# jianing-sun/Mask-YOLO

Measured on AMD Instinct MI355X. Metric: images/sec fwd+bwd, 224x224 Shapes batch 32, at 1 MI355X, higher is better.
Workload: dtype f32

## Files before the change

mask-yolo_amd/csrc/mem_kernels.hip:

```cpp
#include "myolo_common.h"
#include <type_traits>
#include <stdlib.h>
#include <stdarg.h>
#include <string.h>

static thread_local char g_err[512] = "";
extern "C" void myolo_set_error(const char* fmt, ...)
{
    va_list ap;
    va_start(ap, fmt);
    vsnprintf(g_err, sizeof(g_err), fmt, ap);
    va_end(ap);
}
extern "C" const char* myolo_last_error_string(void) { return g_err; }
extern "C" int myolo_version(void) { return 213; }

static MyoloOptions default_options() { MyoloOptions o = {}; o.bn_fused_tf_variance = 1; o.tn_wgs = 224; return o; }
MyoloOptions g_myolo_opt = default_options();
static int* option_slot(const char* name)
{
    static const struct { const char* n; int MyoloOptions::*m; } tab[] = {
        {"gemm_generic", &MyoloOptions::gemm_generic}, {"no_splitk", &MyoloOptions::no_splitk}, {"bf16_no256", &MyoloOptions::bf16_no256},
        {"bf16_force256", &MyoloOptions::bf16_force256}, {"bf16_no_c3", &MyoloOptions::bf16_no_c3}, {"bf16_no_loopn", &MyoloOptions::bf16_no_loopn},
        {"bf16_mask_valu", &MyoloOptions::bf16_mask_valu}, {"bf16_mask_nofin", &MyoloOptions::bf16_mask_nofin},
        {"deconv_mask_legacy", &MyoloOptions::deconv_mask_legacy}, {"crop_bf16_legacy", &MyoloOptions::crop_bf16_legacy},
        {"tune0", &MyoloOptions::tune0}, {"wino_x6", &MyoloOptions::wino_x6}, {"wino_no_bt", &MyoloOptions::wino_no_bt},
        {"wino_no_mixed", &MyoloOptions::wino_no_mixed}, {"x6_no_half_tiles", &MyoloOptions::x6_no_half_tiles},
        {"w63_legacy", &MyoloOptions::w63_legacy}, {"pw_x6_min_rows", &MyoloOptions::pw_x6_min_rows}, {"deconv_no_x6", &MyoloOptions::deconv_no_x6},
        {"pw_no_smallm", &MyoloOptions::pw_no_smallm}, {"pw_no_x6", &MyoloOptions::pw_no_x6}, {"tn_no_x6", &MyoloOptions::tn_no_x6},
        {"tn_wgs", &MyoloOptions::tn_wgs}, {"tn_x6_legacy", &MyoloOptions::tn_x6_legacy}, {"no_trunk_fusion", &MyoloOptions::no_trunk_fusion},
        {"bn_fused_tf_variance", &MyoloOptions::bn_fused_tf_variance},
    };
    if (!name) return nullptr;
    for (const auto& e : tab)
        if (strcmp(e.n, name) == 0) return &(g_myolo_opt.*(e.m));
    return nullptr;
}
extern "C" int myolo_set_option(const char* name, int value)
{
    int* s = option_slot(name);
    MYOLO_REQUIRE(s, "set_option: unknown option '%s'", name ? name : "(null)");
    *s = value;
    return MYOLO_OK;
}
extern "C" int myolo_get_option(const char* name, int* value)
{
    int* s = option_slot(name);
    MYOLO_REQUIRE(s && value, "get_option: unknown option '%s'", name ? name : "(null)");
    *value = *s;
    return MYOLO_OK;
}

#include <vector>
struct WPrepEntry {
    const void* w; int kind; long long d0, d1, d2;
    size_t off, bytes;
    unsigned long long gen;
    unsigned long long last_use;
    std::function<void(void*, hipStream_t)> run;
};
struct WPrep {
    char* arena; size_t cap, used;
    unsigned long long gen;
// ... 3439 lines not shown
```

mask-yolo_amd/csrc/myolo_common.h:

```cpp
#pragma once
#include <hip/hip_runtime.h>
#include <stdint.h>
#include <stdio.h>
#include "../../include/myolo_hip_internal.h"

extern "C" void myolo_set_error(const char* fmt, ...);

struct MyoloOptions {
    int gemm_generic;
    int no_splitk;
    int bf16_no256;
    int bf16_no_loopn;
    int bf16_mask_valu;
    int bf16_mask_nofin;
    int deconv_mask_legacy;
    int bf16_no_c3;
    int bf16_force256;
    int crop_bf16_legacy;
    int tune0;
    int wino_x6;
    int wino_no_bt;
    int wino_no_mixed;
    int x6_no_half_tiles;
    int w63_legacy;
    int pw_x6_min_rows;
    int deconv_no_x6;
    int pw_no_smallm;
    int pw_no_x6;
    int tn_no_x6;
    int tn_wgs;
    int tn_x6_legacy;
    int no_trunk_fusion;
    int bn_fused_tf_variance;
};
extern MyoloOptions g_myolo_opt;

#define MYOLO_REQUIRE(cond, ...)                                   \
    do {                                                           \
        if (!(cond)) {                                             \
            myolo_set_error(__VA_ARGS__);                          \
            return MYOLO_EINVAL;                                   \
        }                                                          \
    } while (0)

#define MYOLO_NEED_WS(bytes)                                                         \
    do {                                                                             \
        if ((size_t)(bytes) > ws_bytes || (ws == nullptr && (bytes) > 0)) {          \
            myolo_set_error("%s: workspace too small (%zu needed, %zu given)",       \
                            __func__, (size_t)(bytes), ws_bytes);                    \
            return MYOLO_EWORKSPACE;                                                 \
        }                                                                            \
    } while (0)

#define MYOLO_CHECK_LAUNCH()                                                         \
    do {                                                                             \
        hipError_t e__ = hipGetLastError();                                          \
        if (e__ != hipSuccess) {                                                     \
            myolo_set_error("%s: launch failed: %s", __func__, hipGetErrorString(e__)); \
            return MYOLO_ELAUNCH;                                                    \
        }                                                                            \
    } while (0)

#include <functional>
enum { WP_TRANSPOSE = 1, WP_X6_SPLIT = 2, WP_WINO63_U = 3, WP_WINO43_U = 4 };
// ... 47 lines not shown
```

mask-yolo_amd/csrc/wino_mm.hip:

```cpp
#include "myolo_common.h"

typedef float f32x16 __attribute__((ext_vector_type(16)));
typedef unsigned int u32x4 __attribute__((ext_vector_type(4)));

#define MM_BM 128
#define MM_BN 256
#define MM_BK 16
#define MM_LD 20
#define MM_OOB 0x7fffff00u

struct MMRun {
    long long rows;
    long long a_off;
    long long b_off;
    long long c_off;
    long long tile0;
    int mtiles;
    int nq;
};
struct MMArgs {
    const float* A;
    const float* Bt;
    float* C;
    int K, N;
// ... 347 lines not shown
            const long long row = m0 + wm * 64 + t * 32 + (r & 3) + 8 * (r >> 2) + 4 * half;
            if (row >= M) continue;
            float* dst = Cp + row * p.N + n0 + wn * 128 + l31;
#pragma unroll
            for (int u = 0; u < 4; ++u) dst[32 * u] = acc[t][u][r];
        }
}

typedef __bf16 bf16x8 __attribute__((ext_vector_type(8)));
#define X6_REC 112

__device__ __forceinline__ unsigned x6_top(float lo, float hi) { return __builtin_amdgcn_perm(__float_as_uint(hi), __float_as_uint(lo), 0x07060302u); }
__device__ __forceinline__ float x6_rest(float x) { return x - __uint_as_float(__float_as_uint(x) & 0xffff0000u); }
__device__ __forceinline__ bf16x8 x6_ldb(__amdgpu_buffer_rsrc_t r, unsigned voff, unsigned soff)
{
    u32x4 v = __builtin_amdgcn_raw_buffer_load_b128(r, (int)voff, (int)soff, 0);
    return __builtin_bit_cast(bf16x8, v);
}

template <int V> struct IntK { static constexpr int value = V; };
template <bool SWAP> __device__ __forceinline__ f32x16 x6_mfma(bf16x8 a, bf16x8 b, f32x16 c)
{
    if constexpr (SWAP) return __builtin_amdgcn_mfma_f32_32x32x16_bf16(b, a, c, 0, 0, 0);
    else return __builtin_amdgcn_mfma_f32_32x32x16_bf16(a, b, c, 0, 0, 0);
}

__device__ __forceinline__ float mm_act(float v, int act)
{
    if (act == MYOLO_ACT_RELU) return fmaxf(v, 0.f);
    if (act == MYOLO_ACT_RELU6) return fminf(fmaxf(v, 0.f), 6.f);
    return v;
}

template <int EPI, bool PW = false, int AG = MM_A_PLAIN, int NU = 4>
__global__ __launch_bounds__(256, 2) void wino_mm_x6_kernel(MMArgs p)
{
    static_assert(NU == 4 || (NU == 2 && EPI == MM_EP_PLAIN && AG == MM_A_PLAIN), "the 128-column tile exists for the plain product only");
    constexpr int BN = 64 * NU;
    __shared__ __attribute__((aligned(16))) unsigned char As[2][MM_BM * X6_REC];
    __shared__ __attribute__((aligned(16))) unsigned char etab[EPI == MM_EP_DECONV_MASK_T ? 5120 + 4096 : 16];

    const int tid = threadIdx.x, lane = tid & 63, wave = tid >> 6;
    const int wm = wave >> 1, wn = wave & 1, half = lane >> 5, l31 = lane & 31;
    const int ntn = p.N / BN;
    long long bid;
    {
        const long long nwg = gridDim.x, orig = blockIdx.x;
        const long long q = nwg >> 3, r = nwg & 7, xcd = orig & 7;
        bid = (xcd < r ? xcd * (q + 1) : r * (q + 1) + (xcd - r) * q) + (orig >> 3);
    }
    int ri = 0;
#pragma unroll
    for (int k = 1; k < 4; ++k)
        if (k < p.nruns && bid >= p.run[k].tile0) ri = k;
    const MMRun& R = p.run[ri];
    const long long local = bid - R.tile0;
    const long long per_plane = (long long)R.mtiles * ntn;
    const int z = (int)(local / per_plane);
    const long long rem = local - z * per_plane;
    const int n0 = (int)(rem % ntn) * BN;
    const long long m0 = (rem / ntn) * MM_BM;
    const long long M = R.rows;
    const int nk = p.K / MM_BK;
    const float* Ap = p.A + R.a_off + (long long)z * M * p.K;
    const unsigned char* Bp = reinterpret_cast<const unsigned char*>(p.Bt) + (R.b_off + (long long)z * p.K * p.N) * 6;
    float* Cp = p.C + R.c_off + (long long)z * M * p.N;
    const long long mend = (m0 + MM_BM < M) ? m0 + MM_BM : M;
    const int arow = tid >> 1, ah = tid & 1;
    __amdgpu_buffer_rsrc_t ra;
    unsigned aoffg;
    unsigned ag_base = 0;
// ... 3 lines not shown
        ra = mm_rsrc(Ap + base_px * p.Co, (end_px - base_px) * p.Co * 4);
        const long long mm = m0 + arow;
        if (mm < M) {
            const long long hw = (long long)p.H * p.W;
            const int rem = (int)(mm - (mm / hw) * hw);
            const int x = rem - (rem / p.W) * p.W;
            ag_base = (unsigned)((4 * mm - 2 * x - base_px) * p.Co + ah * 8) * 4u;
        } else ag_base = MM_OOB;
        aoffg = ag_base;
    } else {
        ra = mm_rsrc(Ap + m0 * p.K, (mend - m0) * p.K * 4);
        aoffg = ((unsigned)arow * (unsigned)p.K + (unsigned)ah * 8u) * 4u;
    }
    const __amdgpu_buffer_rsrc_t rb = mm_rsrc(reinterpret_cast<const float*>(Bp), (long long)p.K * p.N * 6);
    int ag_k = 0;
    const int asto = arow * X6_REC + ah * 16;
    float4 sa[2];
    float4 psc[2], psh[2];
    int kch = ah * 8;
    auto gload = [&]() {
        if constexpr (AG == MM_A_DECONV) {
            const int tap = ag_k / p.Co, c0 = ag_k - tap * p.Co;
            const unsigned sh = (unsigned)(((tap >> 1) * 2 * p.W + (tap & 1)) * p.Co + c0) * 4u;
            aoffg = ag_base == MM_OOB ? MM_OOB : ag_base + sh;
            ag_k += MM_BK;
        }
        sa[0] = mm_bufld4(ra, aoffg);
        sa[1] = mm_bufld4(ra, aoffg == MM_OOB ? MM_OOB : aoffg + 16u);
#ifdef MM_X6_TUNE
        if constexpr (AG == MM_A_PLAIN) { if (!(p.tune & 16)) aoffg += MM_BK * 4u; }
#else
        if constexpr (AG == MM_A_PLAIN) aoffg += MM_BK * 4u;
#endif
        if (PW && p.a_scale) {
            psc[0] = *reinterpret_cast<const float4*>(p.a_scale + kch); psc[1] = *reinterpret_cast<const float4*>(p.a_scale + kch + 4);
            psh[0] = *reinterpret_cast<const float4*>(p.a_shift + kch); psh[1] = *reinterpret_cast<const float4*>(p.a_shift + kch + 4);
            kch += MM_BK;
        }
    };
    auto affine = [&]() {
        if (PW && p.a_scale) {
            sa[0].x = mm_act(fmaf(sa[0].x, psc[0].x, psh[0].x), p.a_act); sa[0].y = mm_act(fmaf(sa[0].y, psc[0].y, psh[0].y), p.a_act);
            sa[0].z = mm_act(fmaf(sa[0].z, psc[0].z, psh[0].z), p.a_act); sa[0].w = mm_act(fmaf(sa[0].w, psc[0].w, psh[0].w), p.a_act);
            sa[1].x = mm_act(fmaf(sa[1].x, psc[1].x, psh[1].x), p.a_act); sa[1].y = mm_act(fmaf(sa[1].y, psc[1].y, psh[1].y), p.a_act);
            sa[1].z = mm_act(fmaf(sa[1].z, psc[1].z, psh[1].z), p.a_act); sa[1].w = mm_act(fmaf(sa[1].w, psc[1].w, psh[1].w), p.a_act);
        }
    };
    auto sstore = [&](int buf) {
        affine();
        const float x[8] = {sa[0].x, sa[0].y, sa[0].z, sa[0].w, sa[1].x, sa[1].y, sa[1].z, sa[1].w};
        float r1[8], r2[8];
#pragma unroll
        for (int e = 0; e < 8; ++e) { r1[e] = x6_rest(x[e]); r2[e] = x6_rest(r1[e]); }
        u32x4 p1, p2, p3;
#pragma unroll
        for (int e = 0; e < 4; ++e) {
            p1[e] = x6_top(x[2 * e], x[2 * e + 1]);
            p2[e] = x6_top(r1[2 * e], r1[2 * e + 1]);
            p3[e] = x6_top(r2[2 * e], r2[2 * e + 1]);
        }
        *reinterpret_cast<u32x4*>(As[buf] + asto) = p1;
        *reinterpret_cast<u32x4*>(As[buf] + asto + 32) = p2;
        *reinterpret_cast<u32x4*>(As[buf] + asto + 64) = p3;
    };
    const int afr = (wm * 64 + l31) * X6_REC + half * 16;
    const unsigned bvo = (unsigned)(((n0 + wn * 32 * NU) >> 5) * 6 + half) * 512u + (unsigned)l31 * 16u;
    const unsigned bchunk = (unsigned)(p.N >> 5) * 3072u;
    unsigned bso = 0;
    bf16x8 bq[NU][3];

    f32x16 acc[2][NU];
#pragma unroll
    for (int t = 0; t < 2; ++t)
#pragma unroll
        for (int u = 0; u < NU; ++u)
#pragma unroll
            for (int r = 0; r < 16; ++r) acc[t][u][r] = 0.f;

    gload();
#pragma unroll
    for (int u = 0; u < NU; ++u)
#pragma unroll
        for (int pc = 0; pc < 3; ++pc) bq[u][pc] = x6_ldb(rb, bvo + u * 3072u + pc * 1024u, bso);
    sstore(0);
    if (nk > 1) gload();
    if constexpr (EPI == MM_EP_DECONV_MASK_T) mm_deconv_mask_table(p, etab, n0, tid);
    __syncthreads();
    bf16x8 fa[2][3];
#pragma unroll
    for (int pc = 0; pc < 3; ++pc) fa[0][pc] = *reinterpret_cast<const bf16x8*>(As[0] + afr + pc * 32);

    if constexpr (NU == 2 && AG == MM_A_PLAIN && EPI == MM_EP_PLAIN) {
        float4 qa[3][2], qsc[3][2], qsh[3][2];
        bf16x8 qb[2][NU][3];
        const float* csc = (PW && p.a_scale) ? p.a_scale : p.A;
        const float* csh = (PW && p.a_scale) ? p.a_shift : p.A;
        const bool has_aff = PW && p.a_scale;
        auto gstage = [&](auto st, bool valid) {
            constexpr int S = decltype(st)::value;
#ifdef MM_X6_TUNE
            if (!(p.tune & 2048)) {
#endif
            qa[S][0] = mm_bufld4(ra, valid ? aoffg : MM_OOB);
            qa[S][1] = mm_bufld4(ra, valid ? aoffg + 16u : MM_OOB);
#ifdef MM_X6_TUNE
            }
#endif
            aoffg += MM_BK * 4u;
#ifdef MM_X6_TUNE
            if (p.tune & 8192) return;
#endif
            if constexpr (PW) {
                const int kc = (valid && has_aff) ? kch : ah * 8;
                qsc[S][0] = *reinterpret_cast<const float4*>(csc + kc); qsc[S][1] = *reinterpret_cast<const float4*>(csc + kc + 4);
                qsh[S][0] = *reinterpret_cast<const float4*>(csh + kc); qsh[S][1] = *reinterpret_cast<const float4*>(csh + kc + 4);
                kch += MM_BK;
            }
        };
        qa[1][0] = sa[0]; qa[1][1] = sa[1];
        if constexpr (PW) { qsc[1][0] = psc[0]; qsc[1][1] = psc[1]; qsh[1][0] = psh[0]; qsh[1][1] = psh[1]; }
#pragma unroll
        for (int u = 0; u < NU; ++u)
#pragma unroll
            for (int pc = 0; pc < 3; ++pc) {
                qb[0][u][pc] = bq[u][pc];
                qb[1][u][pc] = x6_ldb(rb, bvo + u * 3072u + pc * 1024u, nk > 1 ? bchunk : 0u);
            }
        gstage(IntK<2>{}, nk > 2);
        gstage(IntK<0>{}, nk > 3);
        auto step = [&](auto ic, int c) {
            constexpr int I = decltype(ic)::value;
            constexpr int cur = I & 1, SA = (I + 1) % 3, SB = I & 1;
            const bool more = c + 1 < nk;
#ifdef MM_X6_TUNE
            if (!(p.tune & 16384))
#endif
#pragma unroll
            for (int pc = 0; pc < 3; ++pc) fa[1][pc] = *reinterpret_cast<const bf16x8*>(As[cur] + afr + 32 * X6_REC + pc * 32);
            float x[8] = {qa[SA][0].x, qa[SA][0].y, qa[SA][0].z, qa[SA][0].w, qa[SA][1].x, qa[SA][1].y, qa[SA][1].z, qa[SA][1].w};
            if constexpr (PW) {
                if (has_aff) {
                    const float sc8[8] = {qsc[SA][0].x, qsc[SA][0].y, qsc[SA][0].z, qsc[SA][0].w, qsc[SA][1].x, qsc[SA][1].y, qsc[SA][1].z, qsc[SA][1].w};
                    const float sh8[8] = {qsh[SA][0].x, qsh[SA][0].y, qsh[SA][0].z, qsh[SA][0].w, qsh[SA][1].x, qsh[SA][1].y, qsh[SA][1].z, qsh[SA][1].w};
#pragma unroll
                    for (int e = 0; e < 8; ++e) x[e] = mm_act(fmaf(x[e], sc8[e], sh8[e]), p.a_act);
                }
            }
            gstage(IntK<SA>{}, c + 4 < nk);
            const unsigned b2 = c + 2 < nk ? bso + 2u * bchunk : bso;
            u32x4 p1, p2, p3;
            bf16x8 fn0, fn1, fn2;
#pragma unroll
            for (int u = 0; u < NU; ++u) {
#ifdef MM_X6_TUNE
#define X6_GO (!(p.tune & 512))
#else
#define X6_GO true
#endif
#define X6_TILE(t)  if (X6_GO) {                                                                                         \
                acc[t][u] = __builtin_amdgcn_mfma_f32_32x32x16_bf16(fa[t][0], qb[SB][u][2], acc[t][u], 0, 0, 0);       \
                acc[t][u] = __builtin_amdgcn_mfma_f32_32x32x16_bf16(fa[t][2], qb[SB][u][0], acc[t][u], 0, 0, 0);       \
                acc[t][u] = __builtin_amdgcn_mfma_f32_32x32x16_bf16(fa[t][1], qb[SB][u][1], acc[t][u], 0, 0, 0);       \
                acc[t][u] = __builtin_amdgcn_mfma_f32_32x32x16_bf16(fa[t][0], qb[SB][u][1], acc[t][u], 0, 0, 0);       \
                acc[t][u] = __builtin_amdgcn_mfma_f32_32x32x16_bf16(fa[t][1], qb[SB][u][0], acc[t][u], 0, 0, 0);       \
                acc[t][u] = __builtin_amdgcn_mfma_f32_32x32x16_bf16(fa[t][0], qb[SB][u][0], acc[t][u], 0, 0, 0); }
                X6_TILE(0)
                X6_TILE(1)
#undef X6_TILE
#undef X6_GO
#ifdef MM_X6_TUNE
                if (!(p.tune & 1024))
#endif
#pragma unroll
// ... 25 lines not shown
                    if (more && !(p.tune & 16384)) {
#else
                    if (more) {
#endif
                        fn0 = *reinterpret_cast<const bf16x8*>(As[cur ^ 1] + afr);
                        fn1 = *reinterpret_cast<const bf16x8*>(As[cur ^ 1] + afr + 32);
                        fn2 = *reinterpret_cast<const bf16x8*>(As[cur ^ 1] + afr + 64);
                    }
                }
                __builtin_amdgcn_sched_barrier(0);
            }
            if (more) { fa[0][0] = fn0; fa[0][1] = fn1; fa[0][2] = fn2; }
            bso = more ? bso + bchunk : bso;
        };
        int c0 = 0;
        for (; c0 + 6 <= nk; c0 += 6) {
            step(IntK<0>{}, c0); step(IntK<1>{}, c0 + 1); step(IntK<2>{}, c0 + 2);
            step(IntK<3>{}, c0 + 3); step(IntK<4>{}, c0 + 4); step(IntK<5>{}, c0 + 5);
        }
        if (c0 < nk) step(IntK<0>{}, c0);
        if (c0 + 1 < nk) step(IntK<1>{}, c0 + 1);
        if (c0 + 2 < nk) step(IntK<2>{}, c0 + 2);
        if (c0 + 3 < nk) step(IntK<3>{}, c0 + 3);
        if (c0 + 4 < nk) step(IntK<4>{}, c0 + 4);
    } else
    for (int c = 0; c < nk; ++c) {
        const int cur = c & 1;
        const bool more = c + 1 < nk;
#ifdef MM_X6_TUNE
        if (!(p.tune & 64))
#endif
#pragma unroll
        for (int pc = 0; pc < 3; ++pc) fa[1][pc] = *reinterpret_cast<const bf16x8*>(As[cur] + afr + 32 * X6_REC + pc * 32);
        affine();
        const float x[8] = {sa[0].x, sa[0].y, sa[0].z, sa[0].w, sa[1].x, sa[1].y, sa[1].z, sa[1].w};
        u32x4 p1, p2, p3;
#ifdef MM_X6_TUNE
        if (c + 2 < nk && !(p.tune & 128)) gload();
#else
        if (c + 2 < nk) gload();
#endif
#ifdef MM_X6_TUNE
        const unsigned bnext = (p.tune & 1) ? 0u : (more ? bso + bchunk : bso);
#else
        const unsigned bnext = more ? bso + bchunk : bso;
#endif
        bf16x8 fn0, fn1, fn2;
#pragma unroll
        for (int u = 0; u < NU; ++u) {
#define X6_TILE(t)                                                                                                 \
            if (X6_ALL) {                                                                                          \
            acc[t][u] = x6_mfma<EPI == MM_EP_DECONV_MASK_T>(fa[t][0], bq[u][2], acc[t][u]);           \
            acc[t][u] = x6_mfma<EPI == MM_EP_DECONV_MASK_T>(fa[t][2], bq[u][0], acc[t][u]);           \
            acc[t][u] = x6_mfma<EPI == MM_EP_DECONV_MASK_T>(fa[t][1], bq[u][1], acc[t][u]); }         \
            acc[t][u] = x6_mfma<EPI == MM_EP_DECONV_MASK_T>(fa[t][0], bq[u][1], acc[t][u]);           \
            acc[t][u] = x6_mfma<EPI == MM_EP_DECONV_MASK_T>(fa[t][1], bq[u][0], acc[t][u]);           \
            acc[t][u] = x6_mfma<EPI == MM_EP_DECONV_MASK_T>(fa[t][0], bq[u][0], acc[t][u]);
#ifdef MM_X6_TUNE
#define X6_ALL (!(p.tune & 256))
#else
#define X6_ALL true
#endif
            X6_TILE(0)
            X6_TILE(1)
#undef X6_TILE
#undef X6_ALL
#ifdef MM_X6_TUNE
// ... 315 lines not shown
    }
    MYOLO_CHECK_LAUNCH();
    return MYOLO_OK;
}

#define TN_T 256
struct TNRun {
    long long rows;
    long long a_off, b_off;
    long long rows_per_split;
    long long unit0;
    int plane0;
    int nq;
    int splits;
};
struct TNArgs {
    const float* a_scale;
    const float* a_shift;
    int a_act;
    int gH, gW, gCo;
    const float* A;
    const float* B;
    float* part;
    float* C;
    int Ka, N;
    int nruns;
    int tiles_k, tiles_n;
    long long nunits;
    long long unit_base;
    int tune;
    TNRun run[4];
};

template <bool AG = false, bool UNI = true>
__global__ __launch_bounds__(512, 1) void wino_tn_x6_kernel(TNArgs p)
{
    __shared__ __attribute__((aligned(16))) unsigned char Ls[2][2][TN_T * X6_REC];

    const int tid = threadIdx.x, lane = tid & 63, wave = tid >> 6;
    const int wm = wave >> 2, wn = wave & 3, half = lane >> 5, l31 = lane & 31;
    const int ntile = p.tiles_k * p.tiles_n;
  const long long bid = p.unit_base + blockIdx.x;
  {
    const long long pair = bid / ntile;
    const int tile = (int)(bid - pair * ntile);
    const int kat = tile / p.tiles_n, nt = tile - kat * p.tiles_n;
    int ri = 0;
#pragma unroll
    for (int k = 1; k < 4; ++k)
        if (k < p.nruns && pair >= p.run[k].unit0) ri = k;
    const TNRun& R = p.run[ri];
    const long long local = pair - R.unit0;
    const int z = (int)(local / R.splits), sp = (int)(local - (long long)z * R.splits);
    const long long r0 = (long long)sp * R.rows_per_split;
    long long r1 = r0 + R.rows_per_split;
    if (r1 > R.rows) r1 = R.rows;
    const long long nrows = r1 > r0 ? r1 - r0 : 0;
    const int nk = (int)((nrows + MM_BK - 1) / MM_BK);

    const int op = UNI ? __builtin_amdgcn_readfirstlane(tid >> 8) : tid >> 8, col = tid & 255;
    const int ld = op ? p.N : p.Ka;
    const float* base = op ? p.B + R.b_off + ((long long)z * R.rows + r0) * p.N + nt * TN_T
                           : p.A + R.a_off + ((long long)z * R.rows + r0) * p.Ka + kat * TN_T;
    __amdgpu_buffer_rsrc_t rs = mm_rsrc(base, (nrows * ld - (op ? nt : kat) * TN_T) * 4);
    unsigned voff = (unsigned)col * 4u;
    const unsigned rowb = (unsigned)ld * 4u;
    unsigned soff = 0;
    long long g_m = r0, g_base_px = 0;
    int g_x = 0;
// ... 9 lines not shown
    }
    float st[16];
    auto gload = [&]() {
        if (AG && op == 0) {
            int xk = g_x;
#pragma unroll
            for (int k = 0; k < 16; ++k) {
                const long long m = g_m + k;
                const unsigned so = m < r1 ? (unsigned)((4 * m - 2 * xk - g_base_px) * p.gCo) * 4u : MM_OOB;
                st[k] = __uint_as_float(__builtin_amdgcn_raw_buffer_load_b32(rs, (int)(so == MM_OOB ? MM_OOB : voff + so), 0, 0));
                if (++xk == p.gW) xk = 0;
            }
            g_m += 16;
            g_x = xk;
            return;
        }
#ifdef MM_X6_TUNE
        if (p.tune & 1) {
#pragma unroll
            for (int k = 0; k < 16; ++k) st[k] = __uint_as_float(__builtin_amdgcn_raw_buffer_load_b32(rs, (int)MM_OOB, 0, 0));
            return;
        }
        if (p.tune & 16) {
#pragma unroll
            for (int k = 0; k < 16; ++k) st[k] = __uint_as_float(__builtin_amdgcn_raw_buffer_load_b32(rs, (int)voff, (int)((unsigned)k * rowb), 0));
            return;
        }
#endif
#pragma unroll
        for (int k = 0; k < 16; ++k) st[k] = __uint_as_float(__builtin_amdgcn_raw_buffer_load_b32(rs, (int)voff, (int)(soff + (unsigned)k * rowb), 0));
        soff += 16u * rowb;
    };
    unsigned char* const wbase = &Ls[0][op][col * X6_REC];
    const bool pro = p.a_scale != nullptr && op == 0;
    const float csc = pro ? p.a_scale[kat * TN_T + col] : 1.f, csh = pro ? p.a_shift[kat * TN_T + col] : 0.f;
    long long rows_staged = 0;
    auto split_store = [&](int buf, int h) {
        u32x4 p1, p2, p3;
        if (pro) {
#pragma unroll
            for (int j = 0; j < 8; ++j)
                if (rows_staged + 8 * h + j < nrows) st[8 * h + j] = mm_act(fmaf(st[8 * h + j], csc, csh), p.a_act);
        }
#pragma unroll
        for (int e = 0; e < 4; ++e) {
            const float a0 = st[8 * h + 2 * e], a1 = st[8 * h + 2 * e + 1];
#ifdef MM_X6_TUNE
            if (p.tune & 2) { p1[e] = x6_top(a0, a1); p2[e] = p1[e]; p3[e] = p1[e]; continue; }
#endif
            const float b0 = x6_rest(a0), b1 = x6_rest(a1);
            p1[e] = x6_top(a0, a1);
            p2[e] = x6_top(b0, b1);
            p3[e] = x6_top(x6_rest(b0), x6_rest(b1));
        }
#ifdef MM_X6_TUNE
        if (p.tune & 8) return;
#endif
        unsigned char* w = wbase + buf * (2 * TN_T * X6_REC) + h * 16;
        *reinterpret_cast<u32x4*>(w) = p1;
        *reinterpret_cast<u32x4*>(w + 32) = p2;
        *reinterpret_cast<u32x4*>(w + 64) = p3;
    };
    const int afr = (wm * 128 + l31) * X6_REC + half * 16;
    const int bfr = (wn * 64 + l31) * X6_REC + half * 16;

    f32x16 acc[4][2];
#pragma unroll
    for (int t = 0; t < 4; ++t)
#pragma unroll
        for (int u = 0; u < 2; ++u)
#pragma unroll
            for (int r = 0; r < 16; ++r) acc[t][u][r] = 0.f;

    if (nk > 0) {
        gload();
        split_store(0, 0);
        split_store(0, 1);
        if (nk > 1) gload();
    }
    __syncthreads();
    for (int c = 0; c < nk; ++c) {
        const int cur = c & 1;
        const bool more = c + 1 < nk;
        rows_staged = (long long)(c + 1) * MM_BK;
        const unsigned char* la = &Ls[cur][0][0];
        const unsigned char* lb = &Ls[cur][1][0];
        bf16x8 fb[2][3], fa[3], fn[3];
#pragma unroll
        for (int u = 0; u < 2; ++u)
#pragma unroll
            for (int pc = 0; pc < 3; ++pc) fb[u][pc] = *reinterpret_cast<const bf16x8*>(lb + bfr + u * 32 * X6_REC + pc * 32);
#pragma unroll
        for (int pc = 0; pc < 3; ++pc) fa[pc] = *reinterpret_cast<const bf16x8*>(la + afr + pc * 32);
#pragma unroll
        for (int t = 0; t < 4; ++t) {
            if (t < 3) {
#pragma unroll
                for (int pc = 0; pc < 3; ++pc) fn[pc] = *reinterpret_cast<const bf16x8*>(la + afr + (t + 1) * 32 * X6_REC + pc * 32);
            }
#ifdef MM_X6_TUNE
            if (!(p.tune & 4))
#endif
#pragma unroll
            for (int u = 0; u < 2; ++u) {
                acc[t][u] = __builtin_amdgcn_mfma_f32_32x32x16_bf16(fa[0], fb[u][2], acc[t][u], 0, 0, 0);
                acc[t][u] = __builtin_amdgcn_mfma_f32_32x32x16_bf16(fa[2], fb[u][0], acc[t][u], 0, 0, 0);
                acc[t][u] = __builtin_amdgcn_mfma_f32_32x32x16_bf16(fa[1], fb[u][1], acc[t][u], 0, 0, 0);
                acc[t][u] = __builtin_amdgcn_mfma_f32_32x32x16_bf16(fa[0], fb[u][1], acc[t][u], 0, 0, 0);
                acc[t][u] = __builtin_amdgcn_mfma_f32_32x32x16_bf16(fa[1], fb[u][0], acc[t][u], 0, 0, 0);
                acc[t][u] = __builtin_amdgcn_mfma_f32_32x32x16_bf16(fa[0], fb[u][0], acc[t][u], 0, 0, 0);
            }
            if (t == 0 && more) split_store(cur ^ 1, 0);
            if (t == 1 && more) split_store(cur ^ 1, 1);
            if (t == 2 && c + 2 < nk) gload();
            if (t < 3) { fa[0] = fn[0]; fa[1] = fn[1]; fa[2] = fn[2]; }
        }
        __syncthreads();
    }
    float* Pp = p.part + pair * (long long)p.Ka * p.N + ((long long)kat * TN_T + wm * 128) * p.N + nt * TN_T + wn * 64 + l31;
#pragma unroll
    for (int t = 0; t < 4; ++t)
#pragma unroll
        for (int r = 0; r < 16; ++r) {
            const int row = t * 32 + (r & 3) + 8 * (r >> 2) + 4 * half;
#pragma unroll
            for (int u = 0; u < 2; ++u) Pp[(long long)row * p.N + u * 32] = acc[t][u][r];
        }
  }
}

__global__ __launch_bounds__(256) void tn_x6_reduce_kernel(TNArgs p)
{
    const int plane = blockIdx.y;
    int ri = 0;
#pragma unroll
    for (int k = 1; k < 4; ++k)
        if (k < p.nruns && plane >= p.run[k].plane0) ri = k;
    const TNRun& R = p.run[ri];
    const long long n4 = (long long)p.Ka * p.N / 4;
    const long long i = (long long)blockIdx.x * 256 + threadIdx.x;
    if (i >= n4) return;
    const float4* src = reinterpret_cast<const float4*>(p.part) + (R.unit0 + (long long)(plane - R.plane0) * R.splits) * n4 + i;
    float4 s = make_float4(0.f, 0.f, 0.f, 0.f);
    int k = 0;
    for (; k + 4 <= R.splits; k += 4) {
        const float4 a = src[(long long)k * n4], b = src[(long long)(k + 1) * n4], c = src[(long long)(k + 2) * n4], d = src[(long long)(k + 3) * n4];
        s.x += a.x; s.y += a.y; s.z += a.z; s.w += a.w;
        s.x += b.x; s.y += b.y; s.z += b.z; s.w += b.w;
        s.x += c.x; s.y += c.y; s.z += c.z; s.w += c.w;
        s.x += d.x; s.y += d.y; s.z += d.z; s.w += d.w;
// ... 14 lines not shown
    for (int r = 0; r < nruns; ++r) total_rows += rows[r] * nq[r];
    const long long target_units = 3 * (g_myolo_opt.tn_wgs > 0 ? g_myolo_opt.tn_wgs : 256);
    long long rps = ((total_rows * ntile + target_units - 1) / target_units + MM_BK - 1) / MM_BK * MM_BK;
    if (rps < 8 * MM_BK) rps = 8 * MM_BK;
    long long pairs = 0;
    for (int iter = 0; iter < 64; ++iter) {
        pairs = 0;
        for (int r = 0; r < nruns; ++r) pairs += (long long)nq[r] * ((rows[r] + rps - 1) / rps);
        if (pairs * ntile <= target_units || rps >= total_rows) break;
        rps += MM_BK;
    }
    if (a) {
        long long unit = 0;
        int plane = 0;
        a->nruns = 0;
        for (int r = 0; r < nruns; ++r) {
            if (rows[r] <= 0 || nq[r] <= 0) continue;
            TNRun& R = a->run[a->nruns++];
            R.rows = rows[r]; R.nq = nq[r]; R.plane0 = plane; R.unit0 = unit;
            R.splits = (int)((rows[r] + rps - 1) / rps);
            R.rows_per_split = ((rows[r] + R.splits - 1) / R.splits + MM_BK - 1) / MM_BK * MM_BK;
            unit += (long long)R.nq * R.splits;
            plane += nq[r];
        }
    }
    return pairs;
}

static long long tn_x6_grid(long long nunits) { return g_myolo_opt.tn_wgs > 0 && nunits > g_myolo_opt.tn_wgs ? g_myolo_opt.tn_wgs : nunits; }

template <bool AG>
static void tn_x6_launch(TNArgs& a, hipStream_t s)
{
    for (long long base = 0, g = tn_x6_grid(a.nunits); base < a.nunits; base += g) {
        a.unit_base = base;
        const unsigned n = (unsigned)(a.nunits - base < g ? a.nunits - base : g);
        if (g_myolo_opt.tn_x6_legacy) hipLaunchKernelGGL((wino_tn_x6_kernel<AG, false>), dim3(n), dim3(512), 0, s, a);
        else hipLaunchKernelGGL((wino_tn_x6_kernel<AG, true>), dim3(n), dim3(512), 0, s, a);
    }
}

size_t myolo_gemm_tn_x6_ws_bytes(int nruns, const long long* rows, const int* nq, int Ka, int N)
{
    return align256((size_t)tn_x6_plan(nruns, rows, nq, Ka, N, nullptr) * Ka * N * sizeof(float));
}

int myolo_gemm_tn_x6_runs(const float* A, const float* B, float* C, int nruns, const long long* rows, const long long* a_off, const long long* b_off,
                          const int* nq, int Ka, int N, void* part, size_t part_bytes, hipStream_t s,
                          const float* a_scale, const float* a_shift, int a_act)
{
    if (nruns < 0 || nruns > 4 || Ka < TN_T || (Ka % TN_T) || N < TN_T || (N % TN_T) || ((uintptr_t)A & 15) || ((uintptr_t)B & 15) || ((uintptr_t)C & 15)) {
        myolo_set_error("gemm_tn_x6_runs: needs Ka %% %d == 0, N %% %d == 0, <= 4 runs, 16-byte aligned operands", TN_T, TN_T);
        return MYOLO_EINVAL;
    }
    TNArgs a{};
    a.A = A; a.B = B; a.C = C; a.part = (float*)part; a.Ka = Ka; a.N = N; a.tiles_k = Ka / TN_T; a.tiles_n = N / TN_T;
    a.a_scale = a_scale; a.a_shift = a_shift; a.a_act = a_act;
    const long long pairs = tn_x6_plan(nruns, rows, nq, Ka, N, &a);
    if ((size_t)pairs * Ka * N * sizeof(float) > part_bytes || !part) {
        myolo_set_error("gemm_tn_x6_runs: workspace too small (%zu needed, %zu given)", (size_t)pairs * Ka * N * sizeof(float), part_bytes);
        return MYOLO_EWORKSPACE;
    }
    int k = 0, planes = 0;
    for (int r = 0; r < nruns; ++r) {
        if (rows[r] <= 0 || nq[r] <= 0) continue;
        if ((a_off[r] | b_off[r]) & 3) { myolo_set_error("gemm_tn_x6_runs: run offsets must be multiples of 4 elements"); return MYOLO_EINVAL; }
        a.run[k].a_off = a_off[r]; a.run[k].b_off = b_off[r];
        planes += nq[r];
        ++k;
    }
    if (pairs <= 0) return MYOLO_OK;
    a.nunits = pairs * a.tiles_k * a.tiles_n;
#ifdef MM_X6_TUNE
    a.tune = g_myolo_opt.tune0;
#endif
    tn_x6_launch<false>(a, s);
    const long long n4 = (long long)Ka * N / 4;
    hipLaunchKernelGGL(tn_x6_reduce_kernel, dim3((unsigned)((n4 + 255) / 256), planes), dim3(256), 0, s, a);
    return MYOLO_OK;
}

extern "C" int myolo_gemm_tn_bf16x6_planes(const float* A, const float* B, float* C, int nruns, const int64_t* rows, const int32_t* nq, int Ka, int N,
                                           void* ws, size_t ws_bytes, void* stream)
{
    MYOLO_REQUIRE(A && B && C && rows && nq && nruns >= 0 && nruns <= 4 && Ka > 0 && N > 0, "gemm_tn_bf16x6_planes: bad arguments");
    long long r[4], ao[4], bo[4], at = 0;
    int q[4];
    for (int k = 0; k < nruns; ++k) {
        MYOLO_REQUIRE(rows[k] >= 0 && nq[k] >= 0, "gemm_tn_bf16x6_planes: negative run");
        r[k] = rows[k]; q[k] = nq[k]; ao[k] = at * Ka; bo[k] = at * N;
        at += rows[k] * nq[k];
    }
    const int rc = myolo_gemm_tn_x6_runs(A, B, C, nruns, r, ao, bo, q, Ka, N, ws, ws_bytes, (hipStream_t)stream);
    if (rc) return rc;
    MYOLO_CHECK_LAUNCH();
    return MYOLO_OK;
}

bool myolo_pw_x6_ok(int K, int N) { return g_myolo_opt.wino_x6 && !g_myolo_opt.pw_no_x6 && K >= 256 && (K % MM_BK) == 0 && (N % MM_BN) == 0; }
size_t myolo_pw_x6_split_bytes(int K, int N) { return align256((size_t)K * N * 6); }
int myolo_pw_x6_fwd(const float* x, const float* in_scale, const float* in_shift, int in_act, const float* w, float* y, double* stat,
                    long long M, int K, int N, void* split, hipStream_t s)
{
    MMArgs a{};
    a.A = x; a.C = y; a.K = K; a.N = N; a.nruns = 1;
    a.a_scale = in_scale; a.a_shift = in_shift; a.a_act = in_act; a.stat = stat;
#ifdef MM_X6_TUNE
    a.tune = g_myolo_opt.tune0;
#endif
    MMRun& R = a.run[0];
    R.rows = M; R.a_off = 0; R.b_off = 0; R.c_off = 0; R.nq = 1; R.tile0 = 0;
    R.mtiles = (int)((M + MM_BM - 1) / MM_BM);
    const long long tiles = (long long)R.mtiles * (N / MM_BN);
    a.Bt = x6_split_weights(w, split, K, N, 1, s);
    if (x6_half_tiles(tiles)) hipLaunchKernelGGL((wino_mm_x6_kernel<MM_EP_PLAIN, true, MM_A_PLAIN, 2>), dim3((unsigned)(2 * tiles)), dim3(256), 0, s, a);
    else hipLaunchKernelGGL((wino_mm_x6_kernel<MM_EP_PLAIN, true>), dim3((unsigned)tiles), dim3(256), 0, s, a);
    return MYOLO_OK;
}


bool myolo_deconv_x6_ok(int Cin, int Co, int which)
{
    if (!g_myolo_opt.wino_x6 || g_myolo_opt.deconv_no_x6) return false;
    return which == 0 ? ((Cin % MM_BK) == 0 && Cin >= MM_BK && (Co % MM_BN) == 0) : ((Co % MM_BK) == 0 && (Cin % MM_BN) == 0);
}
int myolo_deconv_x6_fwd(const float* x, const float* w, const float* bias, float* y, long long M, int H, int W, int Cin, int Co, int act,
                        void* split, hipStream_t s)
{
    const int K = Cin, N = 4 * Co;
    MMArgs a{};
    a.A = x; a.C = y; a.K = K; a.N = N; a.nruns = 1; a.bias = bias; a.H = H; a.W = W; a.Co = Co; a.a_act = act;
#ifdef MM_X6_TUNE
    a.tune = g_myolo_opt.tune0;
#endif
    MMRun& R = a.run[0];
    R.rows = M; R.nq = 1; R.mtiles = (int)((M + MM_BM - 1) / MM_BM);
    a.Bt = x6_split_weights(w, split, K, N, 0, s);
    hipLaunchKernelGGL((wino_mm_x6_kernel<MM_EP_DECONV, false, MM_A_PLAIN>), dim3((unsigned)((long long)R.mtiles * (N / MM_BN))), dim3(256), 0, s, a);
    return MYOLO_OK;
}
int myolo_deconv_x6_bwd_data(const float* dy, const float* w, float* dx, long long M, int H, int W, int Cin, int Co, void* split, hipStream_t s)
{
    const int K = 4 * Co, N = Cin;
    MMArgs a{};
    a.A = dy; a.C = dx; a.K = K; a.N = N; a.nruns = 1; a.H = H; a.W = W; a.Co = Co;
#ifdef MM_X6_TUNE
    a.tune = g_myolo_opt.tune0;
#endif
    MMRun& R = a.run[0];
// ... 46 lines not shown
```

Measured before the change: 1666.

## Specialize x6 pointwise and TN kernels on compile-time activation with LDS-staged affine

Adds an ACT template parameter to the pointwise x6 GEMM and TN x6 kernels so the on-load BN affine and activation are resolved at compile time instead of through runtime branches. The pointwise kernel now stages scale and shift for all K into shared memory once per block rather than reloading float4 pairs from global memory each chunk. The TN kernel splits its main loop into steady-state and tail chunks so the ragged-row check is skipped in the steady state. The cost is more template instantiations, extra LDS use (up to 16KB), and a K<=2048 limit for the new pointwise path.

After: 1679, median of 6. About the same (+0.8%).

```diff
diff --git a/mask-yolo_amd/csrc/mem_kernels.hip b/mask-yolo_amd/csrc/mem_kernels.hip
--- a/mask-yolo_amd/csrc/mem_kernels.hip
+++ b/mask-yolo_amd/csrc/mem_kernels.hip
@@ -28,7 +28,7 @@
         {"wino_no_mixed", &MyoloOptions::wino_no_mixed}, {"x6_no_half_tiles", &MyoloOptions::x6_no_half_tiles},
         {"w63_legacy", &MyoloOptions::w63_legacy}, {"pw_x6_min_rows", &MyoloOptions::pw_x6_min_rows}, {"deconv_no_x6", &MyoloOptions::deconv_no_x6},
         {"pw_no_smallm", &MyoloOptions::pw_no_smallm}, {"pw_no_x6", &MyoloOptions::pw_no_x6}, {"tn_no_x6", &MyoloOptions::tn_no_x6},
-        {"tn_wgs", &MyoloOptions::tn_wgs}, {"tn_x6_legacy", &MyoloOptions::tn_x6_legacy}, {"no_trunk_fusion", &MyoloOptions::no_trunk_fusion},
+        {"tn_wgs", &MyoloOptions::tn_wgs}, {"tn_x6_legacy", &MyoloOptions::tn_x6_legacy}, {"pw_x6_legacy", &MyoloOptions::pw_x6_legacy},{"no_trunk_fusion", &MyoloOptions::no_trunk_fusion},
         {"bn_fused_tf_variance", &MyoloOptions::bn_fused_tf_variance},
     };
     if (!name) return nullptr;
diff --git a/mask-yolo_amd/csrc/myolo_common.h b/mask-yolo_amd/csrc/myolo_common.h
--- a/mask-yolo_amd/csrc/myolo_common.h
+++ b/mask-yolo_amd/csrc/myolo_common.h
@@ -30,6 +30,7 @@
     int tn_no_x6;
     int tn_wgs;
     int tn_x6_legacy;
+    int pw_x6_legacy;
     int no_trunk_fusion;
     int bn_fused_tf_variance;
 };
diff --git a/mask-yolo_amd/csrc/wino_mm.hip b/mask-yolo_amd/csrc/wino_mm.hip
--- a/mask-yolo_amd/csrc/wino_mm.hip
+++ b/mask-yolo_amd/csrc/wino_mm.hip
@@ -403,11 +403,25 @@
     return v;
 }
 
-template <int EPI, bool PW = false, int AG = MM_A_PLAIN, int NU = 4>
+#define MM_ACT_RT (-2)
+#define MM_ACT_OFF (-1)
+#define MM_AFF_MAXK 2048
+template <int ACT> __device__ __forceinline__ float mm_act_c(float v)
+{
+    if constexpr (ACT == MYOLO_ACT_RELU) return fmaxf(v, 0.f);
+    else if constexpr (ACT == MYOLO_ACT_RELU6) return fminf(fmaxf(v, 0.f), 6.f);
+    else return v;
+}
+
+template <int EPI, bool PW = false, int AG = MM_A_PLAIN, int NU = 4, int ACT = MM_ACT_RT>
 __global__ __launch_bounds__(256, 2) void wino_mm_x6_kernel(MMArgs p)
 {
     static_assert(NU == 4 || (NU == 2 && EPI == MM_EP_PLAIN && AG == MM_A_PLAIN), "the 128-column tile exists for the plain product only");
+    static_assert(PW || ACT == MM_ACT_RT, "the compile-time on-load affine belongs to the pointwise product");
     constexpr int BN = 64 * NU;
+    constexpr bool RT = PW && ACT == MM_ACT_RT;
+    constexpr bool AFF = PW && ACT >= 0;
+    __shared__ __attribute__((aligned(16))) float aff[AFF ? 2 : 1][AFF ? MM_AFF_MAXK : 4];
     __shared__ __attribute__((aligned(16))) unsigned char As[2][MM_BM * X6_REC];
     __shared__ __attribute__((aligned(16))) unsigned char etab[EPI == MM_EP_DECONV_MASK_T ? 5120 + 4096 : 16];
 
@@ -477,14 +491,28 @@
 #else
         if constexpr (AG == MM_A_PLAIN) aoffg += MM_BK * 4u;
 #endif
-        if (PW && p.a_scale) {
+        if (RT && p.a_scale) {
             psc[0] = *reinterpret_cast<const float4*>(p.a_scale + kch); psc[1] = *reinterpret_cast<const float4*>(p.a_scale + kch + 4);
             psh[0] = *reinterpret_cast<const float4*>(p.a_shift + kch); psh[1] = *reinterpret_cast<const float4*>(p.a_shift + kch + 4);
             kch += MM_BK;
         }
     };
-    auto affine = [&]() {
-        if (PW && p.a_scale) {
+    auto aff_apply = [&](float (&x)[8], int chunk) {
+        const float4* sc = reinterpret_cast<const float4*>(&aff[0][chunk * MM_BK + ah * 8]);
+        const float4* sh = reinterpret_cast<const float4*>(&aff[AFF ? 1 : 0][chunk * MM_BK + ah * 8]);
+        const float4 c0 = sc[0], c1 = sc[1], h0 = sh[0], h1 = sh[1];
+        const float sc8[8] = {c0.x, c0.y, c0.z, c0.w, c1.x, c1.y, c1.z, c1.w};
+        const float sh8[8] = {h0.x, h0.y, h0.z, h0.w, h1.x, h1.y, h1.z, h1.w};
+#pragma unroll
+        for (int e = 0; e < 8; ++e) x[e] = mm_act_c<ACT>(fmaf(x[e], sc8[e], sh8[e]));
+    };
+    auto affine = [&](int chunk) {
+        if constexpr (AFF) {
+            float x[8] = {sa[0].x, sa[0].y, sa[0].z, sa[0].w, sa[1].x, sa[1].y, sa[1].z, sa[1].w};
+            aff_apply(x, chunk);
+            sa[0] = make_float4(x[0], x[1], x[2], x[3]); sa[1] = make_float4(x[4], x[5], x[6], x[7]);
+        }
+        if (RT && p.a_scale) {
             sa[0].x = mm_act(fmaf(sa[0].x, psc[0].x, psh[0].x), p.a_act); sa[0].y = mm_act(fmaf(sa[0].y, psc[0].y, psh[0].y), p.a_act);
             sa[0].z = mm_act(fmaf(sa[0].z, psc[0].z, psh[0].z), p.a_act); sa[0].w = mm_act(fmaf(sa[0].w, psc[0].w, psh[0].w), p.a_act);
             sa[1].x = mm_act(fmaf(sa[1].x, psc[1].x, psh[1].x), p.a_act); sa[1].y = mm_act(fmaf(sa[1].y, psc[1].y, psh[1].y), p.a_act);
@@ -492,7 +520,7 @@
         }
     };
     auto sstore = [&](int buf) {
-        affine();
+        affine(0);
         const float x[8] = {sa[0].x, sa[0].y, sa[0].z, sa[0].w, sa[1].x, sa[1].y, sa[1].z, sa[1].w};
         float r1[8], r2[8];
 #pragma unroll
@@ -522,11 +550,22 @@
 #pragma unroll
             for (int r = 0; r < 16; ++r) acc[t][u][r] = 0.f;
 
+    if constexpr (AFF) {
+        float fs[MM_AFF_MAXK / 256], fh[MM_AFF_MAXK / 256];
+#pragma unroll
+        for (int i = 0; i < MM_AFF_MAXK / 256; ++i)
+            if (i * 256 < p.K) { const int k = i * 256 + tid < p.K ? i * 256 + tid : p.K - 1; fs[i] = p.a_scale[k]; fh[i] = p.a_shift[k]; }
+        gload();
+#pragma unroll
+        for (int i = 0; i < MM_AFF_MAXK / 256; ++i)
+            if (i * 256 + tid < p.K) { aff[0][i * 256 + tid] = fs[i]; aff[AFF ? 1 : 0][i * 256 + tid] = fh[i]; }
+    } else
     gload();
 #pragma unroll
     for (int u = 0; u < NU; ++u)
 #pragma unroll
         for (int pc = 0; pc < 3; ++pc) bq[u][pc] = x6_ldb(rb, bvo + u * 3072u + pc * 1024u, bso);
+    if constexpr (AFF) __syncthreads();
     sstore(0);
     if (nk > 1) gload();
     if constexpr (EPI == MM_EP_DECONV_MASK_T) mm_deconv_mask_table(p, etab, n0, tid);
@@ -538,9 +577,9 @@
     if constexpr (NU == 2 && AG == MM_A_PLAIN && EPI == MM_EP_PLAIN) {
         float4 qa[3][2], qsc[3][2], qsh[3][2];
         bf16x8 qb[2][NU][3];
-        const float* csc = (PW && p.a_scale) ? p.a_scale : p.A;
-        const float* csh = (PW && p.a_scale) ? p.a_shift : p.A;
-        const bool has_aff = PW && p.a_scale;
+        const float* csc = (RT && p.a_scale) ? p.a_scale : p.A;
+        const float* csh = (RT && p.a_scale) ? p.a_shift : p.A;
+        const bool has_aff = RT && p.a_scale;
         auto gstage = [&](auto st, bool valid) {
             constexpr int S = decltype(st)::value;
 #ifdef MM_X6_TUNE
@@ -555,7 +594,7 @@
 #ifdef MM_X6_TUNE
             if (p.tune & 8192) return;
 #endif
-            if constexpr (PW) {
+            if constexpr (RT) {
                 const int kc = (valid && has_aff) ? kch : ah * 8;
                 qsc[S][0] = *reinterpret_cast<const float4*>(csc + kc); qsc[S][1] = *reinterpret_cast<const float4*>(csc + kc + 4);
                 qsh[S][0] = *reinterpret_cast<const float4*>(csh + kc); qsh[S][1] = *reinterpret_cast<const float4*>(csh + kc + 4);
@@ -563,7 +602,7 @@
             }
         };
         qa[1][0] = sa[0]; qa[1][1] = sa[1];
-        if constexpr (PW) { qsc[1][0] = psc[0]; qsc[1][1] = psc[1]; qsh[1][0] = psh[0]; qsh[1][1] = psh[1]; }
+        if constexpr (RT) { qsc[1][0] = psc[0]; qsc[1][1] = psc[1]; qsh[1][0] = psh[0]; qsh[1][1] = psh[1]; }
 #pragma unroll
         for (int u = 0; u < NU; ++u)
 #pragma unroll
@@ -583,7 +622,8 @@
 #pragma unroll
             for (int pc = 0; pc < 3; ++pc) fa[1][pc] = *reinterpret_cast<const bf16x8*>(As[cur] + afr + 32 * X6_REC + pc * 32);
             float x[8] = {qa[SA][0].x, qa[SA][0].y, qa[SA][0].z, qa[SA][0].w, qa[SA][1].x, qa[SA][1].y, qa[SA][1].z, qa[SA][1].w};
-            if constexpr (PW) {
+            if constexpr (AFF) aff_apply(x, more ? c + 1 : c);
+            if constexpr (RT) {
                 if (has_aff) {
                     const float sc8[8] = {qsc[SA][0].x, qsc[SA][0].y, qsc[SA][0].z, qsc[SA][0].w, qsc[SA][1].x, qsc[SA][1].y, qsc[SA][1].z, qsc[SA][1].w};
                     const float sh8[8] = {qsh[SA][0].x, qsh[SA][0].y, qsh[SA][0].z, qsh[SA][0].w, qsh[SA][1].x, qsh[SA][1].y, qsh[SA][1].z, qsh[SA][1].w};
@@ -675,7 +715,7 @@
 #endif
 #pragma unroll
         for (int pc = 0; pc < 3; ++pc) fa[1][pc] = *reinterpret_cast<const bf16x8*>(As[cur] + afr + 32 * X6_REC + pc * 32);
-        affine();
+        affine(more ? c + 1 : c);
         const float x[8] = {sa[0].x, sa[0].y, sa[0].z, sa[0].w, sa[1].x, sa[1].y, sa[1].z, sa[1].w};
         u32x4 p1, p2, p3;
 #ifdef MM_X6_TUNE
@@ -1057,9 +1097,10 @@
     TNRun run[4];
 };
 
-template <bool AG = false, bool UNI = true>
+template <bool AG = false, bool UNI = true, int ACT = MM_ACT_RT>
 __global__ __launch_bounds__(512, 1) void wino_tn_x6_kernel(TNArgs p)
 {
+    static_assert(UNI || ACT == MM_ACT_RT, "the compile-time affine exists for the uniform loader only");
     __shared__ __attribute__((aligned(16))) unsigned char Ls[2][2][TN_T * X6_REC];
 
     const int tid = threadIdx.x, lane = tid & 63, wave = tid >> 6;
@@ -1135,12 +1176,19 @@
         soff += 16u * rowb;
     };
     unsigned char* const wbase = &Ls[0][op][col * X6_REC];
-    const bool pro = p.a_scale != nullptr && op == 0;
+    const bool pro = ACT == MM_ACT_RT ? p.a_scale != nullptr && op == 0 : ACT >= 0 && op == 0;
     const float csc = pro ? p.a_scale[kat * TN_T + col] : 1.f, csh = pro ? p.a_shift[kat * TN_T + col] : 0.f;
     long long rows_staged = 0;
-    auto split_store = [&](int buf, int h) {
+    auto split_store = [&](int buf, int h, bool ragged = true) {
         u32x4 p1, p2, p3;
-        if (pro) {
+        if constexpr (ACT >= 0) {
+            if (pro) {
+#pragma unroll
+                for (int j = 0; j < 8; ++j)
+                    if (!ragged || rows_staged + 8 * h + j < nrows) st[8 * h + j] = mm_act_c<ACT>(fmaf(st[8 * h + j], csc, csh));
+            }
+        }
+        if (ACT == MM_ACT_RT && pro) {
 #pragma unroll
             for (int j = 0; j < 8; ++j)
                 if (rows_staged + 8 * h + j < nrows) st[8 * h + j] = mm_act(fmaf(st[8 * h + j], csc, csh), p.a_act);
@@ -1182,9 +1230,11 @@
         if (nk > 1) gload();
     }
     __syncthreads();
-    for (int c = 0; c < nk; ++c) {
+    auto chunk = [&](int c, auto mode) {
+        constexpr int MODE = decltype(mode)::value;
         const int cur = c & 1;
-        const bool more = c + 1 < nk;
+        const bool more = MODE == 0 ? c + 1 < nk : MODE != 3;
+        const bool more2 = MODE == 0 ? c + 2 < nk : MODE == 1;
         rows_staged = (long long)(c + 1) * MM_BK;
         const unsigned char* la = &Ls[cur][0][0];
         const unsigned char* lb = &Ls[cur][1][0];
@@ -1213,12 +1263,19 @@
                 acc[t][u] = __builtin_amdgcn_mfma_f32_32x32x16_bf16(fa[1], fb[u][0], acc[t][u], 0, 0, 0);
                 acc[t][u] = __builtin_amdgcn_mfma_f32_32x32x16_bf16(fa[0], fb[u][0], acc[t][u], 0, 0, 0);
             }
-            if (t == 0 && more) split_store(cur ^ 1, 0);
-            if (t == 1 && more) split_store(cur ^ 1, 1);
-            if (t == 2 && c + 2 < nk) gload();
+            if (t == 0 && more) split_store(cur ^ 1, 0, MODE != 1);
+            if (t == 1 && more) split_store(cur ^ 1, 1, MODE != 1);
+            if (t == 2 && more2) gload();
             if (t < 3) { fa[0] = fn[0]; fa[1] = fn[1]; fa[2] = fn[2]; }
         }
         __syncthreads();
+    };
+    if constexpr (ACT == MM_ACT_RT) {
+        for (int c = 0; c < nk; ++c) chunk(c, IntK<0>{});
+    } else {
+        for (int c = 0; c + 2 < nk; ++c) chunk(c, IntK<1>{});
+        if (nk > 1) chunk(nk - 2, IntK<2>{});
+        if (nk > 0) chunk(nk - 1, IntK<3>{});
     }
     float* Pp = p.part + pair * (long long)p.Ka * p.N + ((long long)kat * TN_T + wm * 128) * p.N + nt * TN_T + wn * 64 + l31;
 #pragma unroll
@@ -1299,11 +1356,17 @@
 template <bool AG>
 static void tn_x6_launch(TNArgs& a, hipStream_t s)
 {
+    const int act = !a.a_scale ? MM_ACT_OFF : a.a_act == MYOLO_ACT_RELU ? MYOLO_ACT_RELU : a.a_act == MYOLO_ACT_RELU6 ? MYOLO_ACT_RELU6 : MYOLO_ACT_NONE;
     for (long long base = 0, g = tn_x6_grid(a.nunits); base < a.nunits; base += g) {
         a.unit_base = base;
         const unsigned n = (unsigned)(a.nunits - base < g ? a.nunits - base : g);
-        if (g_myolo_opt.tn_x6_legacy) hipLaunchKernelGGL((wino_tn_x6_kernel<AG, false>), dim3(n), dim3(512), 0, s, a);
-        else hipLaunchKernelGGL((wino_tn_x6_kernel<AG, true>), dim3(n), dim3(512), 0, s, a);
+        if (g_myolo_opt.tn_x6_legacy == 1) hipLaunchKernelGGL((wino_tn_x6_kernel<AG, false>), dim3(n), dim3(512), 0, s, a);
+        else if (g_myolo_opt.tn_x6_legacy) hipLaunchKernelGGL((wino_tn_x6_kernel<AG, true>), dim3(n), dim3(512), 0, s, a);
+        else if (act == MM_ACT_OFF) hipLaunchKernelGGL((wino_tn_x6_kernel<AG, true, MM_ACT_OFF>), dim3(n), dim3(512), 0, s, a);
+        else if constexpr (AG) hipLaunchKernelGGL((wino_tn_x6_kernel<AG, true>), dim3(n), dim3(512), 0, s, a);
+        else if (act == MYOLO_ACT_RELU) hipLaunchKernelGGL((wino_tn_x6_kernel<AG, true, MYOLO_ACT_RELU>), dim3(n), dim3(512), 0, s, a);
+        else if (act == MYOLO_ACT_RELU6) hipLaunchKernelGGL((wino_tn_x6_kernel<AG, true, MYOLO_ACT_RELU6>), dim3(n), dim3(512), 0, s, a);
+        else hipLaunchKernelGGL((wino_tn_x6_kernel<AG, true, MYOLO_ACT_NONE>), dim3(n), dim3(512), 0, s, a);
     }
 }
 
@@ -1366,6 +1429,17 @@
 
 bool myolo_pw_x6_ok(int K, int N) { return g_myolo_opt.wino_x6 && !g_myolo_opt.pw_no_x6 && K >= 256 && (K % MM_BK) == 0 && (N % MM_BN) == 0; }
 size_t myolo_pw_x6_split_bytes(int K, int N) { return align256((size_t)K * N * 6); }
+template <int NU>
+static void pw_x6_launch(int act, unsigned grid, const MMArgs& a, hipStream_t s)
+{
+    switch (act) {
+    case MM_ACT_OFF: hipLaunchKernelGGL((wino_mm_x6_kernel<MM_EP_PLAIN, true, MM_A_PLAIN, NU, MM_ACT_OFF>), dim3(grid), dim3(256), 0, s, a); break;
+    case MYOLO_ACT_NONE: hipLaunchKernelGGL((wino_mm_x6_kernel<MM_EP_PLAIN, true, MM_A_PLAIN, NU, MYOLO_ACT_NONE>), dim3(grid), dim3(256), 0, s, a); break;
+    case MYOLO_ACT_RELU: hipLaunchKernelGGL((wino_mm_x6_kernel<MM_EP_PLAIN, true, MM_A_PLAIN, NU, MYOLO_ACT_RELU>), dim3(grid), dim3(256), 0, s, a); break;
+    case MYOLO_ACT_RELU6: hipLaunchKernelGGL((wino_mm_x6_kernel<MM_EP_PLAIN, true, MM_A_PLAIN, NU, MYOLO_ACT_RELU6>), dim3(grid), dim3(256), 0, s, a); break;
+    default: hipLaunchKernelGGL((wino_mm_x6_kernel<MM_EP_PLAIN, true, MM_A_PLAIN, NU, MM_ACT_RT>), dim3(grid), dim3(256), 0, s, a); break;
+    }
+}
 int myolo_pw_x6_fwd(const float* x, const float* in_scale, const float* in_shift, int in_act, const float* w, float* y, double* stat,
                     long long M, int K, int N, void* split, hipStream_t s)
 {
@@ -1380,8 +1454,10 @@
     R.mtiles = (int)((M + MM_BM - 1) / MM_BM);
     const long long tiles = (long long)R.mtiles * (N / MM_BN);
     a.Bt = x6_split_weights(w, split, K, N, 1, s);
-    if (x6_half_tiles(tiles)) hipLaunchKernelGGL((wino_mm_x6_kernel<MM_EP_PLAIN, true, MM_A_PLAIN, 2>), dim3((unsigned)(2 * tiles)), dim3(256), 0, s, a);
-    else hipLaunchKernelGGL((wino_mm_x6_kernel<MM_EP_PLAIN, true>), dim3((unsigned)tiles), dim3(256), 0, s, a);
+    const int act = g_myolo_opt.pw_x6_legacy || K > MM_AFF_MAXK ? MM_ACT_RT
+                  : !in_scale ? MM_ACT_OFF : in_act == MYOLO_ACT_RELU ? MYOLO_ACT_RELU : in_act == MYOLO_ACT_RELU6 ? MYOLO_ACT_RELU6 : MYOLO_ACT_NONE;
+    if (x6_half_tiles(tiles)) pw_x6_launch<2>(act, (unsigned)(2 * tiles), a, s);
+    else pw_x6_launch<4>(act, (unsigned)tiles, a, s);
     return MYOLO_OK;
 }
 
```
